# firedrakeproject/firedrake

Hardware: NVIDIA H100
Metric: assembled DoFs/sec (Poisson CG3, 256^3 hex, 1-form/action) (higher is better)
Workload: dtype f64

## Files before the change

### firedrake_b200/csrc/action_hex.cu

```cuda
#include <stdlib.h>
#include <string.h>

#include "common.cuh"

namespace {

template <int N>
struct HelmParams {
    double *y;
    const double *x;
    const double *coords;
    const int *map0;
    const int *map1;
    const int *collist;
    const int *off0;
    const int *off1;
    int ncols;
    int col0;
    int nlay_items;
    int lay_first, lay_step;
    unsigned nlay_rcp;
    int cdim;
    const long long *rowptr;
    const int *colidx;
    double *vals;
    const int *row_lg;
    const int *col_lg;
    const unsigned short *rank_tab;
    int nvar, nlay_total;
    int chunk;
    int ws_flags;
    int *counter;
    double alpha, beta;
    double B[N * N];
    double Dt[N * N];
    double DtR[N * N];
    double DB[N * N];
    double wq[N];
    double xq[N];
};

template <int N>
struct HelmCoefParams : HelmParams<N> {
    const double *kappa;
};

template <int N>
struct HelmNlParams : HelmCoefParams<N> {
    double dcoef[3];
};

template <bool COEF>
__device__ __forceinline__ double coef_weight(double w, const double *s_kap, int q)
{
    if constexpr (COEF) return w * s_kap[q];
    else return w;
}

template <bool COEF, int NL>
__device__ __forceinline__ double stiff_weight(double w, const double *s_kap, int q, double uq, const double *dcoef)
{
    if constexpr (NL == 1) return w * fma(fma(dcoef[2], uq, dcoef[1]), uq, dcoef[0]);
    else if constexpr (NL == 2) return w;
    else return coef_weight<COEF>(w, s_kap, q);
}

__device__ __forceinline__ double fast_rcp(double x)
{
    double r;
    asm("rcp.approx.ftz.f64 %0, %1;" : "=d"(r) : "d"(x));
    const double e = fma(-x, r, 1.0);
    const double t = fma(e, e, e);
    return fma(r, t, r);
}

template <int N, bool T>
__device__ __forceinline__ void apply_first(const double *M, const double (&in)[N][N],
                                            double (&out)[N][N])
{
#pragma unroll
    for (int i = 0; i < N; i++)
#pragma unroll
        for (int j = 0; j < N; j++) {
            double s = 0.0;
#pragma unroll
            for (int k = 0; k < N; k++) s = fma(T ? M[k * N + i] : M[i * N + k], in[k][j], s);
            out[i][j] = s;
        }
}

template <int N, bool T>
__device__ __forceinline__ void apply_second(const double *M, const double (&in)[N][N],
                                             double (&out)[N][N])
{
#pragma unroll
    for (int i = 0; i < N; i++)
#pragma unroll
        for (int j = 0; j < N; j++) {
            double s = 0.0;
#pragma unroll
            for (int k = 0; k < N; k++) s = fma(T ? M[k * N + j] : M[j * N + k], in[i][k], s);
            out[i][j] = s;
        }
}

template <int N>
__device__ __forceinline__ void to_points_in_place(const double *B, double *sk, bool valid, int t)
{
    double kz[N][N], kt[N][N];
#pragma unroll
    for (int x = 0; x < N; x++)
#pragma unroll
        for (int yy = 0; yy < N; yy++) kz[x][yy] = valid ? sk[(x * N + yy) * N + t] : 0.0;
    apply_first<N, false>(B, kz, kt);
    apply_second<N, false>(B, kt, kz);
#pragma unroll
    for (int x = 0; x < N; x++)
#pragma unroll
        for (int yy = 0; yy < N; yy++) sk[(x * N + yy) * N + t] = kz[x][yy];
    __syncwarp();
#pragma unroll
    for (int x = 0; x < N; x++)
#pragma unroll
        for (int z = 0; z < N; z++) kt[x][z] = sk[(x * N + t) * N + z];
    apply_second<N, false>(B, kt, kz);
#pragma unroll
    for (int x = 0; x < N; x++)
#pragma unroll
        for (int z = 0; z < N; z++) sk[(x * N + t) * N + z] = kz[x][z];
}

template <int N>
struct Tile {
    static constexpr int PAD = (N == 4) ? 0 : ((N * N * N) % 2 == 0 ? 2 : 1);
    static constexpr int STRIDE = N * N * N + PAD;
    double *base;
    int t, r, k[N], cwrot;
    __device__ __forceinline__ Tile(double *warp_smem, int cw, int t_) : t(t_)
    {
        base = warp_smem + cw * STRIDE;
        cwrot = cw;
        if (N == 4) {
            r = (t_ + cw) & 3;
#pragma unroll
            for (int j = 0; j < N; j++) k[j] = (j + cw) & 3;
        } else {
            r = t_;
#pragma unroll
            for (int j = 0; j < N; j++) k[j] = j;
        }
    }
    __device__ __forceinline__ void store_Z(const double (&a)[N][N]) const
    {
#pragma unroll
        for (int x = 0; x < N; x++)
#pragma unroll
            for (int y = 0; y < N; y++) base[(x * N + k[y]) * N + r] = a[x][y];
    }
    __device__ __forceinline__ void load_Z(double (&a)[N][N]) const
    {
#pragma unroll
        for (int x = 0; x < N; x++)
#pragma unroll
            for (int y = 0; y < N; y++) a[x][y] = base[(x * N + k[y]) * N + r];
    }
    __device__ __forceinline__ double *row_Y(int z) const
    {
        const int kz = (N == 4) ? ((z + cwrot) & 3) : z;
        return base + r * N + kz;
    }
    __device__ __forceinline__ double get_Y(int x, int z) const { return base[(x * N + r) * N + k[z]]; }
    __device__ __forceinline__ void put_Y(int x, int z, double v) const { base[(x * N + r) * N + k[z]] = v; }
    __device__ __forceinline__ void store_Y(const double (&a)[N][N]) const
    {
#pragma unroll
        for (int x = 0; x < N; x++)
#pragma unroll
            for (int z = 0; z < N; z++) base[(x * N + r) * N + k[z]] = a[x][z];
    }
    __device__ __forceinline__ void load_Y(double (&a)[N][N]) const
    {
#pragma unroll
        for (int x = 0; x < N; x++)
#pragma unroll
            for (int z = 0; z < N; z++) a[x][z] = base[(x * N + r) * N + k[z]];
    }
};

#ifndef FDB_WARPS
#define FDB_WARPS 4
#endif
#ifdef FDB_NO_STASH
constexpr bool OPT_STASH = false;
#else
constexpr bool OPT_STASH = true;
#endif
template <int N, bool SLIM = false, bool COEF = false>
struct WPC {
    static constexpr int value = (N == 6) ? (COEF ? (SLIM ? 5 : 4) : (SLIM ? 8 : 5)) : FDB_WARPS;
};

__device__ __forceinline__ void cp_async8(void *smem, const void *gmem)
{
    unsigned sa = (unsigned)__cvta_generic_to_shared(smem);
    asm volatile("cp.async.ca.shared.global [%0], [%1], 8;" ::"r"(sa), "l"(gmem));
}
__device__ __forceinline__ void cp_async16(void *smem, const void *gmem)
{
    unsigned sa = (unsigned)__cvta_generic_to_shared(smem);
    asm volatile("cp.async.cg.shared.global [%0], [%1], 16;" ::"r"(sa), "l"(gmem));
}
__device__ __forceinline__ void cp_async_commit() { asm volatile("cp.async.commit_group;" ::: "memory"); }
template <int K>
__device__ __forceinline__ void cp_async_wait()
{
    asm volatile("cp.async.wait_group %0;" ::"n"(K) : "memory");
}

__device__ __forceinline__ void cp_async4(void *smem, const void *gmem)
{
    unsigned sa = (unsigned)__cvta_generic_to_shared(smem);
    asm volatile("cp.async.ca.shared.global [%0], [%1], 4;" ::"r"(sa), "l"(gmem));
}

template <int N, bool SLIM = false, bool COEF = false, int NKAP = 1>
struct WarpSmem {
    static constexpr int CW = 32 / N;
    static constexpr int CWS = (32 % N == 0) ? CW : CW + 1;
    static constexpr int ND = N * N * N;
    static constexpr int US = (N == 4) ? ND + 4 : ((ND % 2) ? ND : ND + 1);
    static constexpr int CS = 26;
    static constexpr int TILE = CWS * Tile<N>::STRIDE;
    static constexpr int UBUF = CWS * US;
    static constexpr int COORD = CWS * CS;
#ifndef FDB_STASH_STRIDE
#define FDB_STASH_STRIDE 28
#endif
    static constexpr int GS = FDB_STASH_STRIDE;
    static constexpr int STASH = (OPT_STASH && N == 4 && !SLIM) ? CWS * GS : 0;
    static constexpr int KAPPA = COEF ? NKAP * CWS * US : 0;
    static constexpr int IDX = SLIM ? 0 : 2 * CWS * US;
    static constexpr int MAPRAW = SLIM ? 3 * 2 * US : CWS * US;
    static constexpr int VIDX = SLIM ? 3 * 2 * 8 : 2 * CWS * 8;
    static constexpr int BYTES =
        (((TILE + UBUF + COORD + STASH + KAPPA) * 8 + (IDX + MAPRAW + VIDX) * 4) + 15) / 16 * 16;
    static constexpr int CTA_BYTES = WPC<N, SLIM, COEF>::value * BYTES + ND * 4 + 32;
};

struct Unit {
    int item;
    int comp;
    int ib;
    int cur, end;
    bool valid;
    int col, layer;
    int src;
    bool lead;
};

template <int N, bool MASS, bool ATOMIC, int MINB, bool MATRIX = false, bool SLIM = false, bool AFFINE = false>
__global__ void __launch_bounds__(WPC<N, SLIM>::value * 32, MINB)
helmholtz_action_kernel(const __grid_constant__ HelmParams<N> P)
{
    constexpr bool COEF = false, ADV = false;
    constexpr int NL = 0;
    [[maybe_unused]] const double *kappa = nullptr;
    [[maybe_unused]] const double *dcoef = nullptr;
#include "action_hex_body.cuh"
}

template <int N, bool MASS, bool ATOMIC, int MINB, bool MATRIX = false, bool SLIM = false>
__global__ void __launch_bounds__(WPC<N, SLIM, true>::value * 32, MINB)
helmholtz_coef_kernel(const __grid_constant__ HelmCoefParams<N> P)
{
    constexpr bool COEF = true, AFFINE = false, ADV = false;
    constexpr int NL = 0;
    const double *kappa = P.kappa;
    [[maybe_unused]] const double *dcoef = nullptr;
#include "action_hex_body.cuh"
}

template <int N, bool MASS, bool ATOMIC, int MINB, bool SLIM = false>
__global__ void __launch_bounds__(WPC<N, SLIM>::value * 32, MINB)
nonlinear_residual_kernel(const __grid_constant__ HelmNlParams<N> P)
{
    constexpr bool COEF = false, MATRIX = false, AFFINE = false, ADV = false;
    constexpr int NL = 1;
    [[maybe_unused]] const double *kappa = nullptr;
    const double *dcoef = P.dcoef;
#include "action_hex_body.cuh"
}

template <int N, bool MASS, bool ATOMIC, int MINB, bool MATRIX = false, bool SLIM = false>
__global__ void __launch_bounds__(WPC<N, SLIM, true>::value * 32, MINB)
nonlinear_jacobian_kernel(const __grid_constant__ HelmNlParams<N> P)
{
    constexpr bool COEF = true, AFFINE = false, ADV = false;
    constexpr int NL = 2;
    const double *kappa = P.kappa;
    const double *dcoef = P.dcoef;
#include "action_hex_body.cuh"
}

template <int N, bool MASS, bool ATOMIC, int MINB, bool MATRIX = false>
__global__ void __launch_bounds__(WPC<N, false, true>::value * 32, MINB)
advection_diffusion_kernel(const __grid_constant__ HelmCoefParams<N> P)
{
    constexpr bool COEF = true, AFFINE = false, SLIM = false, ADV = true;
    constexpr int NL = 0;
    const double *kappa = P.kappa;
    [[maybe_unused]] const double *dcoef = nullptr;
#include "action_hex_body.cuh"
}

#include "action_hex_ws.cuh"

template <int N, bool MASS, bool ATOMIC, int MINB, bool MATRIX = false, bool SLIM = false, bool AFFINE = false,
          bool COEF = false, int NL = 0, bool ADV = false>
int launch_one(int grid_cap_per_sm, cudaStream_t st, HelmNlParams<N> &P, int sm_count)
{
    static_assert(NL == 0 || COEF == (NL == 2), "the Jacobian takes the coefficient layout, the residual not");
    static_assert(!ADV || (COEF && NL == 0 && !SLIM), "advection-diffusion takes the coefficient layout");
    using WS = WarpSmem<N, SLIM, COEF, ADV ? 3 : 1>;
    constexpr int WARPS_PER_CTA = WPC<N, SLIM, COEF>::value;
    constexpr int T = WARPS_PER_CTA * 32;
    auto kern = [] {
        if constexpr (ADV) return advection_diffusion_kernel<N, MASS, ATOMIC, MINB, MATRIX>;
        else if constexpr (NL == 1) return nonlinear_residual_kernel<N, MASS, ATOMIC, MINB, SLIM>;
        else if constexpr (NL == 2) return nonlinear_jacobian_kernel<N, MASS, ATOMIC, MINB, MATRIX, SLIM>;
        else if constexpr (COEF) return helmholtz_coef_kernel<N, MASS, ATOMIC, MINB, MATRIX, SLIM>;
        else return helmholtz_action_kernel<N, MASS, ATOMIC, MINB, MATRIX, SLIM, AFFINE>;
    }();
    static bool configured = false;
    static int occ = 1;
    if (!configured) {
        FDB_CUDA(cudaFuncSetAttribute(kern, cudaFuncAttributeMaxDynamicSharedMemorySize, WS::CTA_BYTES));
        FDB_CUDA(cudaOccupancyMaxActiveBlocksPerMultiprocessor(&occ, kern, T, WS::CTA_BYTES));
        if (occ < 1) occ = 1;
        configured = true;
    }
    const int ncells = P.ncols * P.nlay_items;
    const int nitems = (ncells + WS::CW - 1) / WS::CW;
    int per_sm = occ;
    if (grid_cap_per_sm > 0 && grid_cap_per_sm < per_sm) per_sm = grid_cap_per_sm;
    long long grid = (long long)sm_count * per_sm;
    long long need = (nitems + WARPS_PER_CTA - 1) / WARPS_PER_CTA;
    if (grid > need) grid = need;
    if (grid < 1) grid = 1;
    int chunk = P.nlay_items / WS::CW;
    if (chunk < 8) chunk = 8;
    if (chunk > 64) chunk = 64;
    long long per_warp = nitems / (grid * WARPS_PER_CTA) + 1;
    if (chunk > per_warp / 32 + 1) chunk = (int)(per_warp / 32 + 1);
    static const int chunk_env = getenv("FDB_CHUNK") ? atoi(getenv("FDB_CHUNK")) : 0;
    if (chunk_env > 0) chunk = chunk_env;
    P.chunk = chunk;
    P.nlay_rcp = (unsigned)(0x100000000ull / (unsigned long long)P.nlay_items);
    if (P.nlay_items == 1) P.nlay_rcp = 0xffffffffu;
    FDB_CUDA(cudaMemsetAsync(P.counter, 0, sizeof(int), st));
    if constexpr (NL != 0) kern<<<(int)grid, T, WS::CTA_BYTES, st>>>(P);
    else if constexpr (COEF) kern<<<(int)grid, T, WS::CTA_BYTES, st>>>(static_cast<const HelmCoefParams<N> &>(P));
    else kern<<<(int)grid, T, WS::CTA_BYTES, st>>>(static_cast<const HelmParams<N> &>(P));
    FDB_LAUNCH_CHECK();
    return 0;
}

template <int N>
struct CoefMinB {
    static constexpr int value = (N >= 5) ? 1 : 2;
};

template <int N, bool ATOMIC>
int launch_coef(bool mass, int cap, cudaStream_t st, HelmNlParams<N> &P, int sm_count)
{
    constexpr int MB = CoefMinB<N>::value;
    if (N == 6 && P.nlay_items >= 32 / N) {
        if (mass) return launch_one<N, true, ATOMIC, MB, false, (N == 6), false, true>(cap, st, P, sm_count);
        return launch_one<N, false, ATOMIC, MB, false, (N == 6), false, true>(cap, st, P, sm_count);
    }
    if (mass) return launch_one<N, true, ATOMIC, MB, false, false, false, true>(cap, st, P, sm_count);
    return launch_one<N, false, ATOMIC, MB, false, false, false, true>(cap, st, P, sm_count);
}

template <int N>
struct NlResMinB {
    static constexpr int value = (N == 4) ? 3 : ((N >= 5) ? 1 : 2);
};

template <int N, bool ATOMIC>
int launch_nl(int nl, bool mass, int cap, cudaStream_t st, HelmNlParams<N> &P, int sm_count)
{
    constexpr bool SL = (N == 6);
    const bool slim = SL && P.nlay_items >= 32 / N;
    if (nl == 1) {
        constexpr int MB = NlResMinB<N>::value;
        if (slim) {
            if (mass) return launch_one<N, true, ATOMIC, MB, false, SL, false, false, 1>(cap, st, P, sm_count);
            return launch_one<N, false, ATOMIC, MB, false, SL, false, false, 1>(cap, st, P, sm_count);
        }
        if (mass) return launch_one<N, true, ATOMIC, MB, false, false, false, false, 1>(cap, st, P, sm_count);
        return launch_one<N, false, ATOMIC, MB, false, false, false, false, 1>(cap, st, P, sm_count);
    }
    constexpr int MB = CoefMinB<N>::value;
    if (slim) {
        if (mass) return launch_one<N, true, ATOMIC, MB, false, SL, false, true, 2>(cap, st, P, sm_count);
        return launch_one<N, false, ATOMIC, MB, false, SL, false, true, 2>(cap, st, P, sm_count);
    }
    if (mass) return launch_one<N, true, ATOMIC, MB, false, false, false, true, 2>(cap, st, P, sm_count);
    return launch_one<N, false, ATOMIC, MB, false, false, false, true, 2>(cap, st, P, sm_count);
}

template <int N, bool ATOMIC, bool MATRIX = false>
int launch_adv(bool mass, int cap, cudaStream_t st, HelmNlParams<N> &P, int sm_count)
{
    if constexpr (N <= (MATRIX ? 4 : 5)) {
        constexpr int MB = CoefMinB<N>::value;
        if (mass) return launch_one<N, true, ATOMIC, MB, MATRIX, false, false, true, 0, true>(cap, st, P, sm_count);
        return launch_one<N, false, ATOMIC, MB, MATRIX, false, false, true, 0, true>(cap, st, P, sm_count);
    }
    fdb::set_error("advection_diffusion %s: degree %d not instantiated", MATRIX ? "matrix" : "action", N - 1);
    return 1;
}

inline bool is_adv(const fdb_kernel_s *k) { return k->desc.form == FDB_FORM_ADVECTION_DIFFUSION; }

inline int nl_mode(const fdb_kernel_s *k)
{
    if (k->desc.form == FDB_FORM_NONLINEAR_DIFFUSION) return 1;
    if (k->desc.form == FDB_FORM_NONLINEAR_DIFFUSION_JACOBIAN) return 2;
    return 0;
}

template <int N>
void set_dcoef(const fdb_kernel_s *k, HelmNlParams<N> &P)
{
    for (int i = 0; i < 3; i++) P.dcoef[i] = nl_mode(k) ? k->desc.dcoef[i] : 0.0;
}

template <int N, bool ATOMIC>
int launch_variant(bool mass, int minb, int cap, cudaStream_t st, HelmNlParams<N> &P, int sm_count,
                   bool affine = false)
{
    if (affine && ATOMIC) {
        constexpr int AB = (N == 4) ? 3 : ((N >= 5) ? 1 : 2);
        constexpr bool ASL = (N == 6);
        if (!ASL || P.nlay_items >= 32 / N) {
            if (mass) return launch_one<N, true, true, AB, false, ASL, true>(cap, st, P, sm_count);
            return launch_one<N, false, true, AB, false, ASL, true>(cap, st, P, sm_count);
        }
    }
    if (N == 4 && minb == 3) {
        if (mass) return launch_one<N, true, ATOMIC, (N == 4 ? 3 : 2)>(cap, st, P, sm_count);
        return launch_one<N, false, ATOMIC, (N == 4 ? 3 : 2)>(cap, st, P, sm_count);
    }
    if (N == 4 && minb == 4) {
        if (mass) return launch_one<N, true, ATOMIC, (N == 4 ? 4 : 2)>(cap, st, P, sm_count);
        return launch_one<N, false, ATOMIC, (N == 4 ? 4 : 2)>(cap, st, P, sm_count);
    }
    if (N == 4 && minb == 1) {
        if (mass) return launch_one<N, true, ATOMIC, 1>(cap, st, P, sm_count);
        return launch_one<N, false, ATOMIC, 1>(cap, st, P, sm_count);
    }
    constexpr int DEF = (N >= 5) ? 1 : 2;
    if (N == 6) {
        static const bool slim_on = !(getenv("FDB_NO_SLIM") && atoi(getenv("FDB_NO_SLIM")));
        if (slim_on && P.nlay_items >= 32 / N) {
            if (mass) return launch_one<N, true, ATOMIC, DEF, false, (N == 6)>(cap, st, P, sm_count);
            return launch_one<N, false, ATOMIC, DEF, false, (N == 6)>(cap, st, P, sm_count);
        }
    }
    if (mass) return launch_one<N, true, ATOMIC, DEF>(cap, st, P, sm_count);
    return launch_one<N, false, ATOMIC, DEF>(cap, st, P, sm_count);
}

template <int N>
int launch_n(fdb_kernel_s *k, fdb_int start, fdb_int end, int nlay, const fdb_int *subset,
             double *y, const double *coords, const double *x, const fdb_int *map0,
             const fdb_int *map1, const double *kappa)
{
    fdb::Context &c = fdb::ctx();
    HelmNlParams<N> P;
    P.kappa = kappa;
    set_dcoef(k, P);
    const int nl = nl_mode(k);
    P.y = y;
    P.x = x;
    P.coords = coords;
    P.map0 = map0;
    P.map1 = map1;
    P.off0 = k->d_off0;
    P.off1 = k->d_off1;
    P.cdim = k->desc.cdim;
    P.alpha = k->desc.alpha;
    P.beta = k->desc.beta;
    for (int i = 0; i < N * N; i++) {
        P.B[i] = k->desc.B[i];
        P.Dt[i] = k->Dt[i];
    }
    for (int q = 0; q < N; q++)
        for (int j = 0; j < N; j++) {
            P.DtR[q * N + j] = k->Dt[q * N + (j + q) % N];
            double d = 0.0;
            for (int i = 0; i < N; i++) d += k->Dt[q * N + i] * k->desc.B[i * N + j];
            P.DB[q * N + j] = d;
        }
    for (int i = 0; i < N; i++) {
        P.wq[i] = k->desc.wq[i];
        P.xq[i] = k->desc.xq[i];
    }
    const bool mass = k->desc.beta != 0.0;
    static const int minb = getenv("FDB_MINB") ? atoi(getenv("FDB_MINB")) : 3;
    static const int cap = getenv("FDB_CTAS_PER_SM") ? atoi(getenv("FDB_CTAS_PER_SM")) : 0;
    P.counter = c.work_counter;
    if (k->desc.scatter == FDB_SCATTER_ATOMIC) {
        P.collist = subset;
        P.col0 = start;
        P.ncols = end - start;
        P.nlay_items = nlay;
        P.lay_first = 0;
        P.lay_step = 1;
        if (P.ncols <= 0 || nlay <= 0) return 0;
        if (is_adv(k)) return launch_adv<N, true>(mass, cap, c.stream, P, c.sm_count);
        if (kappa && !nl) return launch_coef<N, true>(mass, cap, c.stream, P, c.sm_count);
        if (nl) return launch_nl<N, true>(nl, mass, cap, c.stream, P, c.sm_count);
        if constexpr (N == 4) {
            static const int ws = getenv("FDB_WS") ? atoi(getenv("FDB_WS")) : 0;
            if (ws && P.cdim == 1 && nlay >= 8 && !k->desc.affine_cells) {
#define FDB_WS_CASE(id, NC, NM, NS, ST)                                                            \
    if (ws == id)                                                                              \
        return mass ? launch_ws<true, NC, NM, NS, ST>(c.stream, P, c.sm_count)                 \
                    : launch_ws<false, NC, NM, NS, ST>(c.stream, P, c.sm_count);
                FDB_WS_CASE(1, 12, 4, 2, true)
                FDB_WS_CASE(2, 8, 4, 3, true)
                FDB_WS_CASE(3, 8, 4, 3, false)
                FDB_WS_CASE(4, 8, 8, 3, false)
#undef FDB_WS_CASE
            }
        }
        return launch_variant<N, true>(mass, minb, cap, c.stream, P, c.sm_count, k->desc.affine_cells != 0);
    }
    if (subset) {
        fdb::set_error("coloured scatter does not support subsets yet");
        return 1;
    }
    for (int col = 0; col < k->ncolours; col++) {
        int cbeg = k->colour_start[col], cend = k->colour_start[col + 1];
        for (int par = 0; par < (nlay > 1 ? 2 : 1); par++) {
            P.collist = k->d_colour_cols + cbeg;
            P.col0 = 0;
            P.ncols = cend - cbeg;
            P.lay_first = par;
            P.lay_step = 2;
            P.nlay_items = (nlay - par + 1) / 2;
            if (P.ncols <= 0 || P.nlay_items <= 0) continue;
            if (is_adv(k)      ? launch_adv<N, false>(mass, cap, c.stream, P, c.sm_count)
                : kappa && !nl ? launch_coef<N, false>(mass, cap, c.stream, P, c.sm_count)
                : nl         ? launch_nl<N, false>(nl, mass, cap, c.stream, P, c.sm_count)
                             : launch_variant<N, false>(mass, minb, cap, c.stream, P, c.sm_count))
                return 1;
        }
    }
    return 0;
}

template <int N>
int launch_matrix_n(fdb_kernel_s *k, fdb_int start, fdb_int end, int nlay, const fdb_int *subset,
                    fdb_mat_t mat, const double *coords, const fdb_int *map0, const fdb_int *map1,
                    double *diag_out, const double *kappa)
{
    fdb::Context &c = fdb::ctx();
    HelmNlParams<N> P;
    memset(&P, 0, sizeof(P));
    P.kappa = kappa;
    set_dcoef(k, P);
    P.coords = coords;
    P.map0 = map0;
    P.map1 = map1;
    P.off0 = k->d_off0;
    P.off1 = k->d_off1;
    P.cdim = N * N * N;
    P.alpha = k->desc.alpha;
    P.beta = k->desc.beta;
    for (int i = 0; i < N * N; i++) {
        P.B[i] = k->desc.B[i];
        P.Dt[i] = k->Dt[i];
    }
    for (int q = 0; q < N; q++)
        for (int j = 0; j < N; j++) {
            P.DtR[q * N + j] = k->Dt[q * N + (j + q) % N];
            double d = 0.0;
            for (int i = 0; i < N; i++) d += k->Dt[q * N + i] * k->desc.B[i * N + j];
            P.DB[q * N + j] = d;
        }
    for (int i = 0; i < N; i++) {
        P.wq[i] = k->desc.wq[i];
        P.xq[i] = k->desc.xq[i];
    }
    if (mat) {
        fdb_mat_device_view(mat, &P.rowptr, &P.colidx, &P.vals, &P.row_lg, &P.col_lg);
        fdb_mat_rank_table(mat, &P.rank_tab, &P.nvar);
    } else {
        P.y = diag_out;
    }
    P.nlay_total = nlay;
    if (subset || k->desc.cell != FDB_CELL_HEX_EXTRUDED) P.rank_tab = nullptr;
    P.counter = c.work_counter;
    P.collist = subset;
    P.col0 = start;
    P.ncols = end - start;
    P.nlay_items = nlay;
    P.lay_first = 0;
    P.lay_step = 1;
    if (P.ncols <= 0 || nlay <= 0) return 0;
    if (is_adv(k)) return launch_adv<N, true, true>(k->desc.beta != 0.0, 0, c.stream, P, c.sm_count);
    if (kappa && nl_mode(k) == 0) {
        constexpr int MB = CoefMinB<N>::value;
        if (k->desc.beta != 0.0)
            return launch_one<N, true, true, MB, true, false, false, true>(0, c.stream, P, c.sm_count);
        return launch_one<N, false, true, MB, true, false, false, true>(0, c.stream, P, c.sm_count);
    }
    if (nl_mode(k) == 2) {
        constexpr int MB = CoefMinB<N>::value;
        if (k->desc.beta != 0.0)
            return launch_one<N, true, true, MB, true, false, false, true, 2>(0, c.stream, P, c.sm_count);
        return launch_one<N, false, true, MB, true, false, false, true, 2>(0, c.stream, P, c.sm_count);
    }
    constexpr int DEF = (N >= 5) ? 1 : 2;
    if (k->desc.beta != 0.0) return launch_one<N, true, true, DEF, true>(0, c.stream, P, c.sm_count);
    return launch_one<N, false, true, DEF, true>(0, c.stream, P, c.sm_count);
}

}

int fdb_launch_helmholtz_matrix(fdb_kernel_s *k, fdb_int start, fdb_int end, int nlay,
                                const fdb_int *subset, fdb_mat_t mat, const double *coords,
                                const fdb_int *map0, const fdb_int *map1, double *diag_out)
{
    const int dmma = fdb_opt_matrix_kernel;
    if (mat && dmma != 0 && k->n1d <= 5 && k->n1d >= (dmma == 1 ? 3 : 4))
        return fdb_launch_helmholtz_matrix_dmma(k, start, end, nlay, subset, mat, coords, map0, map1);
    switch (k->n1d) {
    case 2: return launch_matrix_n<2>(k, start, end, nlay, subset, mat, coords, map0, map1, diag_out, nullptr);
    case 3: return launch_matrix_n<3>(k, start, end, nlay, subset, mat, coords, map0, map1, diag_out, nullptr);
    case 4: return launch_matrix_n<4>(k, start, end, nlay, subset, mat, coords, map0, map1, diag_out, nullptr);
    case 5: return launch_matrix_n<5>(k, start, end, nlay, subset, mat, coords, map0, map1, diag_out, nullptr);
    }
    fdb::set_error("helmholtz matrix: degree %d not instantiated (1..4)", k->n1d - 1);
    return 1;
}

int fdb_launch_helmholtz_action(fdb_kernel_s *k, fdb_int start, fdb_int end, int nlay,
                                const fdb_int *subset, double *y, const double *coords,
                                const double *x, const fdb_int *map0, const fdb_int *map1)
{
    static const bool q1_thread = !(getenv("FDB_Q1_THREAD") && atoi(getenv("FDB_Q1_THREAD")) == 0);
    if (q1_thread && k->n1d == 2 && k->desc.cdim == 1 && k->desc.scatter == FDB_SCATTER_ATOMIC &&
        k->desc.cell == FDB_CELL_HEX_EXTRUDED && nlay >= 16)
        return fdb_launch_q1_action(k, start, end, nlay, subset, y, coords, x, map0, map1);
    static const bool q2_thread = !(getenv("FDB_Q2_THREAD") && atoi(getenv("FDB_Q2_THREAD")) == 0);
    if (q2_thread && k->n1d == 3 && k->desc.cdim == 1 && k->desc.scatter == FDB_SCATTER_ATOMIC &&
        k->desc.cell == FDB_CELL_HEX_EXTRUDED && nlay >= 16)
        return fdb_launch_q2_action(k, start, end, nlay, subset, y, coords, x, map0, map1);
    switch (k->n1d) {
    case 2: return launch_n<2>(k, start, end, nlay, subset, y, coords, x, map0, map1, nullptr);
    case 3: return launch_n<3>(k, start, end, nlay, subset, y, coords, x, map0, map1, nullptr);
    case 4: return launch_n<4>(k, start, end, nlay, subset, y, coords, x, map0, map1, nullptr);
    case 5: return launch_n<5>(k, start, end, nlay, subset, y, coords, x, map0, map1, nullptr);
    case 6: return launch_n<6>(k, start, end, nlay, subset, y, coords, x, map0, map1, nullptr);
    }
    fdb::set_error("helmholtz action: degree %d not instantiated (1..5)", k->n1d - 1);
    return 1;
}

int fdb_launch_helmholtz_coef_action(fdb_kernel_s *k, fdb_int start, fdb_int end, int nlay,
                                     const fdb_int *subset, double *y, const double *coords,
                                     const double *x, const double *kappa, const fdb_int *map0,
                                     const fdb_int *map1)
{
    switch (k->n1d) {
    case 2: return launch_n<2>(k, start, end, nlay, subset, y, coords, x, map0, map1, kappa);
    case 3: return launch_n<3>(k, start, end, nlay, subset, y, coords, x, map0, map1, kappa);
    case 4: return launch_n<4>(k, start, end, nlay, subset, y, coords, x, map0, map1, kappa);
    case 5: return launch_n<5>(k, start, end, nlay, subset, y, coords, x, map0, map1, kappa);
    case 6: return launch_n<6>(k, start, end, nlay, subset, y, coords, x, map0, map1, kappa);
    }
    fdb::set_error("helmholtz_coef action: degree %d not instantiated (1..5)", k->n1d - 1);
    return 1;
}

int fdb_launch_helmholtz_coef_matrix(fdb_kernel_s *k, fdb_int start, fdb_int end, int nlay,
                                     const fdb_int *subset, fdb_mat_t mat, const double *coords,
                                     const double *kappa, const fdb_int *map0, const fdb_int *map1,
                                     double *diag_out)
{
    switch (k->n1d) {
    case 2: return launch_matrix_n<2>(k, start, end, nlay, subset, mat, coords, map0, map1, diag_out, kappa);
    case 3: return launch_matrix_n<3>(k, start, end, nlay, subset, mat, coords, map0, map1, diag_out, kappa);
    case 4: return launch_matrix_n<4>(k, start, end, nlay, subset, mat, coords, map0, map1, diag_out, kappa);
    case 5: return launch_matrix_n<5>(k, start, end, nlay, subset, mat, coords, map0, map1, diag_out, kappa);
    }
    fdb::set_error("helmholtz_coef matrix: degree %d not instantiated (1..4)", k->n1d - 1);
    return 1;
}
```

Before: 33.85 billion.

## Add dedicated CG3 hex action kernel using FP64 DMMA for z-direction contractions

Adds a specialized body for degree-3 (N=4) constant-coefficient hex actions. The z-direction interpolation and gradient contractions are done with m8n8k4 FP64 tensor-core MMAs across each 4-lane group, which replaces shuffles or shared-memory passes. It also restructures the quadrature loop to rotate register tiles per y-plane and interleaves prefetch of the next cell's data. The cost is extra kernel-specific code and a possible change in register pressure and occupancy.

```diff
diff --git a/firedrake_b200/csrc/action_hex.cu b/firedrake_b200/csrc/action_hex.cu
--- a/firedrake_b200/csrc/action_hex.cu
+++ b/firedrake_b200/csrc/action_hex.cu
@@ -104,6 +104,13 @@
         }
 }
 
+__device__ __forceinline__ void dmma_m8n8k4(double &d0, double &d1, double a, double b, double c0, double c1)
+{
+    asm volatile("mma.sync.aligned.m8n8k4.row.col.f64.f64.f64.f64 {%0,%1}, {%2}, {%3}, {%4,%5};"
+                 : "=d"(d0), "=d"(d1)
+                 : "d"(a), "d"(b), "d"(c0), "d"(c1));
+}
+
 template <int N>
 __device__ __forceinline__ void to_points_in_place(const double *B, double *sk, bool valid, int t)
 {
@@ -262,11 +269,15 @@
 __global__ void __launch_bounds__(WPC<N, SLIM>::value * 32, MINB)
 helmholtz_action_kernel(const __grid_constant__ HelmParams<N> P)
 {
-    constexpr bool COEF = false, ADV = false;
-    constexpr int NL = 0;
-    [[maybe_unused]] const double *kappa = nullptr;
-    [[maybe_unused]] const double *dcoef = nullptr;
+    if constexpr (N == 4 && !MATRIX && !SLIM && !AFFINE) {
+#include "action_hex_cg3.cuh"
+    } else {
+        constexpr bool COEF = false, ADV = false;
+        constexpr int NL = 0;
+        [[maybe_unused]] const double *kappa = nullptr;
+        [[maybe_unused]] const double *dcoef = nullptr;
 #include "action_hex_body.cuh"
+    }
 }
 
 template <int N, bool MASS, bool ATOMIC, int MINB, bool MATRIX = false, bool SLIM = false>
diff --git a/firedrake_b200/csrc/action_hex_cg3.cuh b/firedrake_b200/csrc/action_hex_cg3.cuh
--- /dev/null
+++ b/firedrake_b200/csrc/action_hex_cg3.cuh
@@ -0,0 +1,327 @@
+    static_assert(N == 4 && !SLIM && !MATRIX && !AFFINE, "the degree-3 constant-coefficient 1-form");
+    using WS = WarpSmem<N>;
+    static_assert(N * N * 32 <= WS::TILE, "the tile holds N*N own slots per lane");
+    constexpr int CW = WS::CW;
+    constexpr int ND = N * N * N;
+    constexpr int US = WS::US;
+    constexpr int CS = WS::CS;
+    constexpr bool STASH = WS::STASH > 0;
+    extern __shared__ __align__(16) unsigned char smem_raw[];
+    const int lane = threadIdx.x & 31, warp = threadIdx.x >> 5;
+    double *wbase = reinterpret_cast<double *>(smem_raw + (size_t)warp * WS::BYTES);
+    double *s_tile = wbase;
+    double *s_u = s_tile + WS::TILE;
+    double *s_coord = s_u + WS::UBUF;
+    double *s_stash = s_coord + WS::COORD;
+    int *s_idx = reinterpret_cast<int *>(s_stash + WS::STASH);
+    int *s_mapraw = s_idx + WS::IDX;
+    int *s_vidx = s_mapraw + WS::MAPRAW;
+    int *s_off0 = reinterpret_cast<int *>(smem_raw + (size_t)WPC<N>::value * WS::BYTES);
+    int *s_off1 = s_off0 + ND;
+
+    for (int i = threadIdx.x; i < ND; i += blockDim.x) s_off0[i] = P.off0[i];
+    if (threadIdx.x < 8) s_off1[threadIdx.x] = P.off1[threadIdx.x];
+    __syncthreads();
+
+    const int cw = lane >> 2, t = lane & 3;
+    const int ncells = P.ncols * P.nlay_items;
+    const int nitems = (ncells + CW - 1) / CW;
+    const double zeta = P.xq[t];
+    const double wz_alpha = P.wq[t] * P.alpha;
+    const double wz_beta = P.wq[t] * P.beta;
+    const double mf = (cw & 1) ? P.DB[(cw >> 1) * N + t] : P.B[(cw >> 1) * N + t];
+    const double mb = (cw & 1) ? 0.0 : P.B[t * N + (cw >> 1)];
+    const double mdb = (cw & 1) ? 0.0 : P.DB[t * N + (cw >> 1)];
+    double *zt = s_tile + lane;
+
+    auto advance = [&](Unit u) -> Unit {
+        if (u.item >= 0 && u.comp + 1 < P.cdim) {
+            u.comp++;
+            return u;
+        }
+        u.comp = 0;
+        u.ib ^= 1;
+        if (u.item >= 0 && u.cur + 1 < u.end) {
+            u.cur++;
+            u.item = u.cur;
+            return u;
+        }
+        if (u.item == -2) return u;
+        int base = 0;
+        if (lane == 0) base = atomicAdd(P.counter, P.chunk);
+        base = __shfl_sync(0xffffffffu, base, 0);
+        if (base >= nitems) {
+            u.item = -2;
+            return u;
+        }
+        u.cur = base;
+        u.end = min(base + P.chunk, nitems);
+        u.item = base;
+        return u;
+    };
+    auto decode = [&](Unit &u) {
+        const int lin = u.item * CW + cw;
+        u.valid = u.item >= 0 && lin < ncells;
+        unsigned ci = __umulhi((unsigned)lin, P.nlay_rcp);
+        int kk = lin - (int)ci * P.nlay_items;
+        if (kk >= P.nlay_items) { kk -= P.nlay_items; ci++; }
+        if (!u.valid) { ci = 0; kk = 0; }
+        u.layer = P.lay_first + P.lay_step * kk;
+        u.col = P.collist ? __ldg(P.collist + ci) : (P.col0 + (int)ci);
+        const unsigned peers = __match_any_sync(0xffffffffu, u.valid ? u.col : -1 - cw);
+        u.src = (__ffs(peers) - 1) / N;
+        u.lead = u.src == cw;
+    };
+    auto row_of = [&](const Unit &u) -> int * { return s_mapraw + u.src * US; };
+    auto vrow_of = [&](const Unit &u) -> int * { return s_vidx + (u.ib * CW + u.src) * 8; };
+    auto stageA = [&](const Unit &u) {
+        if (u.valid && u.comp == 0 && u.lead) {
+            const int *mrow = P.map0 + (long long)u.col * ND;
+            int *sm = row_of(u);
+            for (int j = t; j < ND / 4; j += N) cp_async16(sm + 4 * j, mrow + 4 * j);
+            int *sv = vrow_of(u);
+            for (int v = t; v < 8; v += N) cp_async4(sv + v, P.map1 + (long long)u.col * 8 + v);
+        }
+    };
+    auto stageB_coords = [&](const Unit &u) {
+        if (u.valid && u.comp == 0) {
+            const int *sv = vrow_of(u);
+            double *scd = s_coord + cw * CS;
+            for (int i = t; i < 24; i += N) {
+                int v = i / 3, a = i - v * 3;
+                int g = sv[v] + s_off1[v] * u.layer;
+                cp_async8(scd + i, P.coords + (long long)g * 3 + a);
+            }
+        }
+    };
+    auto stageB_part = [&](const Unit &u, int part) {
+        if (u.valid) {
+            double *su = s_u + cw * US;
+            int *si = s_idx + (u.ib * CW + cw) * US;
+            const int *sm = row_of(u);
+            int g[N];
+            if (u.comp == 0) {
+#pragma unroll
+                for (int j = 0; j < N; j++) {
+                    const int loc = (part * N + j) * N + t;
+                    g[j] = sm[loc] + s_off0[loc] * u.layer;
+                    si[loc] = g[j];
+                }
+            } else {
+#pragma unroll
+                for (int j = 0; j < N; j++) g[j] = si[(part * N + j) * N + t];
+            }
+#pragma unroll
+            for (int j = 0; j < N; j++)
+                cp_async8(su + (part * N + j) * N + t, P.x + (long long)g[j] * P.cdim + u.comp);
+        }
+    };
+
+    Unit cur{-1, 0, 0, 0, 0, false, 0, 0, 0, false};
+    cur = advance(cur);
+    decode(cur);
+    Unit nxt = advance(cur);
+    decode(nxt);
+    stageA(cur);
+    cp_async_commit();
+    cp_async_wait<0>();
+    __syncwarp();
+    stageB_coords(cur);
+#pragma unroll
+    for (int part = 0; part < N; part++) stageB_part(cur, part);
+    stageA(nxt);
+    cp_async_commit();
+    double A1[3], A3[3], A6[3], c3[3], c5[3], c6[3], c7[3];
+
+    while (cur.item >= 0) {
+        cp_async_wait<0>();
+        __syncwarp();
+        Unit nn = advance(nxt);
+        decode(nn);
+
+        const bool valid = cur.valid;
+        const double *sc = s_coord + cw * CS;
+        if (cur.comp == 0) {
+#pragma unroll
+            for (int a = 0; a < 3; a++) {
+                double X000 = sc[0 * 3 + a], X001 = sc[1 * 3 + a], X010 = sc[2 * 3 + a],
+                       X011 = sc[3 * 3 + a], X100 = sc[4 * 3 + a], X101 = sc[5 * 3 + a],
+                       X110 = sc[6 * 3 + a], X111 = sc[7 * 3 + a];
+                if (!valid) {
+                    X000 = 0; X001 = (a == 2); X010 = (a == 1); X011 = (a >= 1);
+                    X100 = (a == 0); X101 = (a != 1); X110 = (a != 2); X111 = 1;
+                }
+                double c1 = X100 - X000;
+                double c2 = X010 - X000;
+                c3[a] = X001 - X000;
+                double c4 = X110 - X100 - X010 + X000;
+                c5[a] = X011 - X010 - X001 + X000;
+                c6[a] = X101 - X100 - X001 + X000;
+                c7[a] = X111 - X110 - X101 - X011 + X100 + X010 + X001 - X000;
+                A1[a] = fma(c6[a], zeta, c1);
+                A3[a] = fma(c5[a], zeta, c2);
+                A6[a] = fma(c7[a], zeta, c4);
+            }
+        }
+        if (STASH && cur.comp == 0) {
+            double *sg = s_stash + cw * WS::GS;
+            if (t == 0) {
+                double2 *d = reinterpret_cast<double2 *>(sg);
+                d[0] = make_double2(c3[0], c3[1]);
+                d[1] = make_double2(c3[2], c6[0]);
+                d[2] = make_double2(c6[1], c6[2]);
+                d[3] = make_double2(c5[0], c5[1]);
+                d[4] = make_double2(c5[2], c7[0]);
+                d[5] = make_double2(c7[1], c7[2]);
+            }
+            double2 *d = reinterpret_cast<double2 *>(sg + 12 + 4 * t);
+            d[0] = make_double2(A1[0], A1[1]);
+            sg[12 + 4 * t + 2] = A1[2];
+            __syncwarp();
+        }
+        const int comp = cur.comp;
+        const int *si = s_idx + (cur.ib * CW + cw) * US;
+        {
+            const double *su = s_u + cw * US;
+            double u[N][N], tmp[N][N], U[N][N], Vp[N][N];
+#pragma unroll
+            for (int x = 0; x < N; x++)
+#pragma unroll
+                for (int yy = 0; yy < N; yy++) u[x][yy] = valid ? su[(x * N + yy) * N + t] : 0.0;
+            apply_first<N, false>(P.B, u, tmp);
+            apply_second<N, false>(P.B, tmp, u);
+#pragma unroll
+            for (int x = 0; x < N; x++)
+#pragma unroll
+                for (int yy = 0; yy < N; yy++) {
+                    double gz;
+                    dmma_m8n8k4(U[x][yy], gz, u[x][yy], mf, 0.0, 0.0);
+                    zt[(x * N + yy) * 32] = gz;
+                }
+#pragma unroll
+            for (int i = 0; i < N; i++)
+#pragma unroll
+                for (int j = 0; j < N; j++) Vp[i][j] = 0.0;
+            __syncwarp();
+            stageB_coords(nxt);
+#pragma unroll 1
+            for (int qy = 0; qy < N; qy++) {
+                stageB_part(nxt, qy);
+                const double eta = P.xq[qy];
+                double dy[N];
+#pragma unroll
+                for (int j = 0; j < N; j++) dy[j] = P.DtR[qy * N + j];
+                double ca[3], pb[3], qb[3];
+                if (STASH) {
+                    const double *sg = s_stash + cw * WS::GS;
+                    const double2 *d = reinterpret_cast<const double2 *>(sg);
+                    const double2 g0 = d[0], g1 = d[1], g2 = d[2], g3 = d[3], g4 = d[4], g5 = d[5];
+                    const double2 a01 = *reinterpret_cast<const double2 *>(sg + 12 + 4 * t);
+                    const double a2 = sg[12 + 4 * t + 2];
+                    pb[0] = fma(g3.x, eta, g0.x);
+                    pb[1] = fma(g3.y, eta, g0.y);
+                    pb[2] = fma(g4.x, eta, g1.x);
+                    qb[0] = fma(g4.y, eta, g1.y);
+                    qb[1] = fma(g5.x, eta, g2.x);
+                    qb[2] = fma(g5.y, eta, g2.y);
+                    ca[0] = fma(A6[0], eta, a01.x);
+                    ca[1] = fma(A6[1], eta, a01.y);
+                    ca[2] = fma(A6[2], eta, a2);
+                } else {
+#pragma unroll
+                    for (int a = 0; a < 3; a++) {
+                        ca[a] = fma(A6[a], eta, A1[a]);
+                        pb[a] = fma(c5[a], eta, c3[a]);
+                        qb[a] = fma(c7[a], eta, c6[a]);
+                    }
+                }
+                const double wyz_a = wz_alpha * P.wq[qy];
+                const double wyz_b = wz_beta * P.wq[qy];
+                double *zrow = zt + qy * 32;
+#pragma unroll
+                for (int qx = 0; qx < N; qx++) {
+                    const double xi = P.xq[qx];
+                    double cb[3], cc[3];
+#pragma unroll
+                    for (int a = 0; a < 3; a++) {
+                        cb[a] = fma(A6[a], xi, A3[a]);
+                        cc[a] = fma(qb[a], xi, pb[a]);
+                    }
+                    double gx = 0.0, gy = 0.0;
+#pragma unroll
+                    for (int q = 0; q < N; q++) {
+                        gx = fma(P.Dt[qx * N + q], U[q][0], gx);
+                        gy = fma(dy[q], U[qx][q], gy);
+                    }
+                    const double gz = zrow[qx * N * 32];
+                    double r0[3], r1[3], r2[3];
+                    r0[0] = cb[1] * cc[2] - cb[2] * cc[1];
+                    r0[1] = cb[2] * cc[0] - cb[0] * cc[2];
+                    r0[2] = cb[0] * cc[1] - cb[1] * cc[0];
+                    r1[0] = cc[1] * ca[2] - cc[2] * ca[1];
+                    r1[1] = cc[2] * ca[0] - cc[0] * ca[2];
+                    r1[2] = cc[0] * ca[1] - cc[1] * ca[0];
+                    r2[0] = ca[1] * cb[2] - ca[2] * cb[1];
+                    r2[1] = ca[2] * cb[0] - ca[0] * cb[2];
+                    r2[2] = ca[0] * cb[1] - ca[1] * cb[0];
+                    const double det = ca[0] * r0[0] + ca[1] * r0[1] + ca[2] * r0[2];
+                    const double adet = fabs(det);
+                    const double s = wyz_a * P.wq[qx] * fast_rcp(adet);
+                    double h[3];
+#pragma unroll
+                    for (int a = 0; a < 3; a++) h[a] = r0[a] * gx + r1[a] * gy + r2[a] * gz;
+                    const double fx = s * (r0[0] * h[0] + r0[1] * h[1] + r0[2] * h[2]);
+                    const double fy = s * (r1[0] * h[0] + r1[1] * h[1] + r1[2] * h[2]);
+                    const double fz = s * (r2[0] * h[0] + r2[1] * h[1] + r2[2] * h[2]);
+                    zrow[qx * N * 32] = fz;
+#pragma unroll
+                    for (int q = 0; q < N; q++) {
+                        Vp[q][0] = fma(P.Dt[qx * N + q], fx, Vp[q][0]);
+                        Vp[qx][q] = fma(dy[q], fy, Vp[qx][q]);
+                    }
+                    if (MASS) Vp[qx][0] = fma(wyz_b * P.wq[qx] * adet, U[qx][0], Vp[qx][0]);
+                }
+#pragma unroll
+                for (int x = 0; x < N; x++) {
+                    const double u0 = U[x][0], v0 = Vp[x][0];
+#pragma unroll
+                    for (int j = 0; j < N - 1; j++) {
+                        U[x][j] = U[x][j + 1];
+                        Vp[x][j] = Vp[x][j + 1];
+                    }
+                    U[x][N - 1] = u0;
+                    Vp[x][N - 1] = v0;
+                }
+            }
+
+            __syncwarp();
+            stageA(nn);
+            cp_async_commit();
+
+#pragma unroll
+            for (int x = 0; x < N; x++)
+#pragma unroll
+                for (int yy = 0; yy < N; yy++) {
+                    double w0, w1;
+                    dmma_m8n8k4(w0, w1, Vp[x][yy], mb, 0.0, 0.0);
+                    dmma_m8n8k4(w0, w1, zt[(x * N + yy) * 32], mdb, w0, w1);
+                    u[x][yy] = w0;
+                }
+            apply_first<N, true>(P.B, u, tmp);
+            apply_second<N, true>(P.B, tmp, u);
+
+            if (valid) {
+#pragma unroll
+                for (int x = 0; x < N; x++)
+#pragma unroll
+                    for (int yy = 0; yy < N; yy++) {
+                        double *dst = P.y + (long long)si[(x * N + yy) * N + t] * P.cdim + comp;
+                        if (ATOMIC) atomicAdd(dst, u[x][yy]);
+                        else *dst += u[x][yy];
+                    }
+            }
+        }
+        cur = nxt;
+        nxt = nn;
+    }
+    cp_async_wait<0>();
```

Result: faster. 35.10 billion, median of 6 (+3.7%).
